# ywrt/slam-robot

Measured on AMD Instinct MI355X. Metric: local-BA iters/sec (50 KF, 20k pts), higher is better.
Workload: dtype f64

## Files before the change

include/slamgpu.h:

```cpp
#ifndef SLAMGPU_H_
#define SLAMGPU_H_

#include <stddef.h>
#include <stdint.h>

#ifdef __cplusplus
extern "C" {
#endif

#define SG_OK 0
#define SG_EINVAL (-22)
#define SG_ENOMEM (-12)
#define SG_EDEVICE (-5)
#define SG_ENODEV (-19)
#define SG_ECOMM (-71)

enum sg_point_flag {
  SG_BAD_LOCATION = 0,
  SG_NO_BASELINE = 1,
  SG_NO_OBSERVATIONS = 2,
  SG_MISMATCHED = 3,
  SG_BAD_FEATURE = 4
};

// ... 132 lines not shown
int sg_ba_kernel_times(sg_ba* h, char* names, int32_t names_len, double* ms, int32_t* counts, int32_t max);
int sg_ba_kernel_work(sg_ba* h, double* bytes, double* flops, int32_t max);

typedef struct sg_ba_info {
  int32_t num_frames, num_points, num_obs;
  int32_t num_blocks;
  int32_t n;
  int32_t band_tiles;
  int32_t cholesky_path;
  int32_t num_pairs;
  int32_t rank, nranks;
  int32_t cholesky_split;
  int32_t num_allreduces;
  int32_t lin_waves;
  int32_t cholesky_separator;
} sg_ba_info;
int sg_ba_info_get(const sg_ba* h, sg_ba_info* out);

int sg_ba_sweep(sg_ba* h, int32_t n);

int sg_ba_evaluate(sg_ba* h, double* residuals, double* cost, int32_t* num_failed);

typedef struct sg_slam sg_slam;
int sg_slam_create(sg_slam** out, const sg_device_options* dev);
void sg_slam_destroy(sg_slam* s);
int sg_slam_solve_frames(sg_slam* s, sg_map* map, int32_t num_to_solve, int32_t num_to_present,
                         double range, int32_t* solved);
int sg_slam_solve_all_frames(sg_slam* s, sg_map* map, double range, int32_t solve_cameras,
                             int32_t* solved);
int sg_slam_reproject_map(sg_slam* s, sg_map* map, double* mean);
// ... 97 lines not shown
```

slam-robot_amd/csrc/ba_chol.hip:

```cpp
#include "ba_lm.h"
#include "ba_tile.h"

namespace sg {

constexpr int kPanelWaves = 3;

__device__ __forceinline__ double& Wn(double* win, int i, int j) {
  return win[(i & (kCholWS - 1)) * kCholLd + (j & (kCholWS - 1))];
}

__device__ __forceinline__ double readlane_d(double v, int l) {
  const int lo = __builtin_amdgcn_readlane(__double2loint(v), l);
  const int hi = __builtin_amdgcn_readlane(__double2hiint(v), l);
  return __hiloint2double(hi, lo);
}



__device__ __forceinline__ void chol_diag16(double (&col)[kCholNb], int w, int lane, bool& bad) {
#pragma unroll
  for (int j = 0; j < kCholNb; ++j) {
    if (j < w) {
      const double piv = readlane_d(col[j], j);
      if (!(piv > 0.0)) bad = true;
// ... 840 lines not shown

__device__ __forceinline__ double row_sum16(double v) {
  v += dpp_d<0x128>(v);
  v += dpp_d<0x124>(v);
  v += dpp_d<0x122>(v);
  v += dpp_d<0x121>(v);
  return v;
}

struct TileSrc {
  int rev;
  int np;
  int sep;
  int nb;
  int ld;
};

__device__ __forceinline__ f64x4 tile_load(const double* __restrict__ S, int I, int J, int li, int lk,
                                           const TileSrc& ts) {
  f64x4 t;
  const int n = ts.nb, ld = ts.ld;
  const int cz = ld * ld + ld;
  const bool zsep = I >= ts.sep && J >= ts.sep;
#pragma unroll
  for (int q = 0; q < 4; ++q) {
    const int gi = 16 * I + lk + 4 * q, gj = 16 * J + li;
    const int si = ts.rev ? ts.np - 1 - gj : gi, sj = ts.rev ? ts.np - 1 - gi : gj;
    const bool in = I >= 0 && si < n && sj < n && !zsep;
    t[q] = S[in ? si * ld + sj : cz + ((gi == gj && !zsep) ? 1 : 0)];
  }
  return t;
}


__device__ __forceinline__ bool tile_diag(const f64x4& D, double ypart, TileShared& sh, double* zp, int K,
// ... 93 lines not shown
#pragma unroll
    for (int q = 0; q < 4; ++q) st_wt(wg + q * 64, Wt[q]);
  } else {
#pragma unroll
    for (int q = 0; q < 4; ++q) wg[q * 64] = Wt[q];
  }
}

__device__ __forceinline__ void tile_rotate(f64x4 (&acc)[kTB]) {
  const f64x4 t = acc[0];
#pragma unroll
  for (int u = 0; u < kTB - 1; ++u) acc[u] = acc[u + 1];
  acc[kTB - 1] = t;
}

__device__ __forceinline__ void tile_col_load(f64x4 (&acc)[kTB], double& ypart, const Dev& d, int J, int K,
                                              int li, int lk, const TileSrc& ts) {
#pragma unroll
  for (int u = 0; u < kTB; ++u) acc[u] = tile_load(d.S, J - ((J - (u + K - 1)) & 7), J, li, lk, ts);
  const int gj = 16 * J + li, ld = ts.ld;
  const int sj = ts.rev ? ts.np - 1 - gj : gj;
  ypart = d.S[(lk == 0 && sj < ts.nb && J < ts.sep) ? ld * ld + sj : ld * ld + ld];
}

constexpr int kLaSpinMax = 1 << 20;
__device__ __forceinline__ bool la_done(const int* tend, int Kp) {
  return Kp >= 0 && Kp + 2 < tend[Kp];
}

template <bool kStamp>
__device__ __forceinline__ void tile_phase(f64x4 (&acc)[kTB], double& ypart, int& J, bool& late, bool& bad,
                                           bool& tmo, TileShared& sh, const Dev& d,
                                           double* __restrict__ Wg, double* zp, const int* tend, int K, int NT,
                                           int lane, int li, int lk, const TileSrc& ts, double* zg, double* zw,
                                           unsigned long long (&tacc)[16], unsigned long long& tlast) {
  const bool wt = zw != nullptr;
  if (late) {
#ifdef SG_X_NOLATE
    J += kTB;
    late = false;
    return;
#endif
    const bool hasw = J < tend[K - 1];
    f64x4 Wt = {0.0, 0.0, 0.0, 0.0};
    if (hasw) Wt = tile_w(acc[0], sh.Zs[(K - 1) & 3], li, lk);
    SG_AST(0)
    const int Jw = J;
    J += kTB;
#ifndef SG_X_NOLOAD
    tile_col_load(acc, ypart, d, J, K, li, lk, ts);
#endif
    SG_AST(1)
    if (hasw) tile_w_store(Wt, Wg, K - 1, Jw, lane, wt);
    SG_AST(2)
    tile_zp(sh, zp, K, lane, zg, zw);
    SG_AST(3)
    late = false;
    SG_TSTAMP(13)
    return;
  }
  if (J == K + 1) SG_PTRACE(K, 8)
#ifdef SG_X_PRIO
  if (J == K + 1) __builtin_amdgcn_s_setprio(3);
#endif
#ifdef SG_X_IDLE
// ... 332 lines not shown
  int K = K0;
  bool first = true;
  for (; K >= Klo + 2; K -= 4) {
#pragma unroll
    for (int q = 0; q < 4; ++q) zB[q] = zsrc[16 * (K - 2) + lk + 4 * q];
    bs_row(K, wA, zA, first);
    first = false;
#pragma unroll
    for (int q = 0; q < 4; ++q) zA[q] = zsrc[16 * (K >= 4 ? K - 4 : 0) + lk + 4 * q];
    bs_row(K - 2, wB, zB, false);
  }
  if (K >= Klo) bs_row(K, wA, zA, first);
}

constexpr int kSepSpinMax = 1 << 22;
template <bool kStamp>
__global__ __launch_bounds__(kTileThreads) void k_chol_tiles(Dev d, const int32_t* panel_jend,
                                                             double* __restrict__ Wg, int32_t* tflag, int nd,
                                                             int flags) {
  const LmState* st = d.st;
  unsigned long long tlast = kStamp ? __builtin_amdgcn_s_memtime() : 0ull, tacc[16] = {};
  const unsigned long long hstart = tlast;
  unsigned long long hlast = 0ull, hacc[6] = {};
  bool hchain = false;
  __shared__ TileShared sh;
  extern __shared__ double tdyn[];
  const bool border = (flags & 8) != 0;
  const int n = border ? d.kc0 : d.n, tid = threadIdx.x, lane = tid & 63;
  const int wave = __builtin_amdgcn_readfirstlane(tid >> 6);
  const int li = lane & 15, lk = lane >> 4;
  const int NT = (n + 15) >> 4;
  const bool bottom = nd > 0 && blockIdx.x == 1;
  const int nsf = (flags >> 8) & 15;
  const int ns = nsf > 0 && nsf < kTB ? nsf : kTB - 1;
  const int m = nd > 0 ? NT - nd - ns : NT;
  const int NTf = nd > 0 ? (bottom ? nd : m + ns) : NT;
  double* Wb = bottom ? Wg + (size_t)NT * kTB * 256 : Wg;
  double* zpg = Wg + (size_t)2 * NT * kTB * 256;
  double* sepb = zpg + 16 * NT;
  double* sepy = sepb + 49 * 256;
  const TileSrc ts{bottom ? 1 : 0, 16 * NT, bottom ? nd : (1 << 28), n, d.n};
  double* zg = border ? Wb : nullptr;
  double* xs = tdyn;
  double* zp = tdyn + 16 * NT;
  int* tend = reinterpret_cast<int*>(tdyn + 32 * NT);
  int* rdone = tend + NT;
  int* rdone_b = rdone + NT;
  for (int k = tid; k < 2 * NT; k += kTileThreads) rdone[k] = 0;
  const bool cand_lds = (flags & 2) != 0;
  CandLds cl;
  cl.carve(tdyn + 32 * NT + (3 * NT + 1) / 2, d.F, d.D, n);
  const int epoch = nd > 0 ? tflag[bottom ? 0 : 1] : 0;
  if (tid == 0) {
    sh.fail = 0;
    sh.tmo = 0;
    sh.uflag = -1;
  }
  bool bad = false, tmo = false;
  const int spin_max = (flags & 4) ? 256 : kSepSpinMax;
  if (bottom && (flags & 4))
    for (int i = 0; i < 640; ++i) __builtin_amdgcn_s_sleep(127);
  if (bottom && (flags & 64))
    for (int i = 0; i < 16; ++i) __builtin_amdgcn_s_sleep(127);
  const bool zpre_in = (flags & 16) != 0 && !bottom;
  f64x4 D0;
  bool zbad = false;
  if (zpre_in) {
#pragma unroll
    for (int q = 0; q < 4; ++q) D0[q] = d.zpre[(lk + 4 * q) * 16 + li];
    zbad = d.zpre[256] != 0.0;
  } else {
    D0 = tile_load(d.S, 0, 0, li, lk, ts);
  }
  double y0;
  {
    const int sj0 = ts.rev ? ts.np - 1 - li : li, ld = ts.ld;
    y0 = d.S[(lk == 0 && sj0 < n && 0 < ts.sep) ? ld * ld + sj0 : ld * ld + ld];
  }
  const int done = st->done;
  if (lane == 0) sh.simd[wave] = __builtin_amdgcn_s_getreg((1 << 11) | (4 << 6) | 4);
  for (int i = tid; i < 16 * kTLd; i += kTileThreads) sh.Id[i] = (i / kTLd == i % kTLd) ? 1.0 : 0.0;
  lds_barrier();
  int col = wave;
  {
    const int my = sh.simd[wave];
    int cnt[4] = {0, 0, 0, 0}, rank = 0;
#pragma unroll
// ... 2 lines not shown
      cnt[sw] += 1;
      if (w < wave && sw == my) rank += 1;
    }
#ifdef SG_X_PAIR4
    if (cnt[0] == 2 && cnt[1] == 2 && cnt[2] == 2 && cnt[3] == 2) col = my + 4 * rank;
#else
    if (cnt[0] == 2 && cnt[1] == 2 && cnt[2] == 2 && cnt[3] == 2) col = 2 * my + rank;
#endif
  }
  {
    f64x4 acc[kTB];
    double ypart = 0.0;
    int J = col;
    bool late = false;
    if (J == 0) J = kTB;
    tile_col_load(acc, ypart, d, J, 0, li, lk, ts);
    for (int k = tid; k < NT; k += kTileThreads) {
      if (!bottom) {
        tend[k] = min((panel_jend[k] + 15) >> 4, NTf);
      } else {
        const int c = NT - 1 - k;
        int te[kTB];
#pragma unroll
        for (int h = 0; h < kTB; ++h) te[h] = panel_jend[max(0, c - kTB + h)];
        int lo = c;
#pragma unroll
        for (int h = kTB - 1; h >= 0; --h) {
          const int i = c - kTB + h;
          if (i >= 0 && ((te[h] + 15) >> 4) > c) lo = i;
        }
        tend[k] = min(NT - lo, nd + ns);
      }
    }
    if (done) return;
// ... 29 lines not shown
          int spin = 0;
          if (lane == 0)
            while (__hip_atomic_load(tflag, __ATOMIC_RELAXED, __HIP_MEMORY_SCOPE_AGENT) <= epoch &&
                   ++spin < spin_max)
              __builtin_amdgcn_s_sleep(1);
          spin = __builtin_amdgcn_readfirstlane(spin);
          asm volatile("" ::: "memory");
          SG_HSTAMP(0)
          tmo |= spin >= spin_max;
          sep_merge(acc, ypart, J, m, ns, sepb, sepy, lane, li, lk);
          if (kStamp) asm volatile("s_waitcnt vmcnt(0)" ::: "memory");
          SG_HSTAMP(1)
          hchain = J == m;
        }
      }
      tile_phase<kStamp>(acc, ypart, J, late, bad, tmo, sh, d, Wb, zp, tend, K, NTf, lane, li, lk, ts, zg,
                         bottom ? zpg : nullptr, tacc, tlast);
      SG_TSTAMP(2)
      if (!late) tile_rotate(acc);
      SG_PTRACE(K, wave)
#ifdef SG_X_ARRIVE
      if (role == 0) { SG_AST(4) } else if (role == 1) { SG_AST(9) } else { SG_AST(13) }
      if (kStamp) {
        const unsigned long long ta = __builtin_amdgcn_s_memtime() - t_ph;
#pragma unroll
        for (int q = 0; q < 8; ++q)
          if (q == d0) {
            ar_sum[q] += ta;
            ar_max[q] = ar_max[q] > ta ? ar_max[q] : ta;
            ar_cnt[q] += 1;
          }
// ... 398 lines not shown
  }
  __syncthreads();
  if (cand_lds)
    chol_candidates_lds<kBordThreads>(d, xs, bad_sh, cl, st->cur, tmo_sh);
  else
    chol_candidates<kBordThreads>(d, xs, bad_sh, tmo_sh);
  if (d.stamps && tid == 0) {
    bstamp(4);
#pragma unroll
    for (int k = 1; k < 10; ++k) d.stamps[48 + k - 1] += tst[k] - tst[0];
  }
}



static const void* const kCholTilesKernels[] = {(const void*)k_chol_tiles<false>, (const void*)k_chol_tiles<true>};

void CholSetAttributes(size_t* tile_lds, size_t* gchol_lds, size_t* border_lds) {
  SG_HIP_CHECK(hipFuncSetAttribute((const void*)k_cholesky_window<false>,
                                   hipFuncAttributeMaxDynamicSharedMemorySize, (int)kCholLds));
  SG_HIP_CHECK(hipFuncSetAttribute((const void*)k_cholesky_window<true>,
                                   hipFuncAttributeMaxDynamicSharedMemorySize, (int)kCholLds));
  size_t lim = 160 * 1024;
  for (const void* f : kCholTilesKernels) {
    hipFuncAttributes fa;
    SG_HIP_CHECK(hipFuncGetAttributes(&fa, f));
    lim = std::min(lim, (size_t)160 * 1024 - fa.sharedSizeBytes);
  }
  for (const void* f : kCholTilesKernels)
    SG_HIP_CHECK(hipFuncSetAttribute(f, hipFuncAttributeMaxDynamicSharedMemorySize, (int)lim));
  *tile_lds = lim;
// ... 7 lines not shown
    hipFuncAttributes ba;
    SG_HIP_CHECK(hipFuncGetAttributes(&ba, f));
    blim = std::min(blim, (size_t)160 * 1024 - ba.sharedSizeBytes);
  }
  SG_REQUIRE(border_lds_doubles(kTileMaxNT, 0, 0, 0, 0) * sizeof(double) <= blim, SG_EINVAL,
             "k_chol_border: LDS for kTileMaxNT rows");
  for (const void* f : {(const void*)k_chol_border<true>, (const void*)k_chol_border<false>})
    SG_HIP_CHECK(hipFuncSetAttribute(f, hipFuncAttributeMaxDynamicSharedMemorySize, (int)blim));
  *border_lds = blim;
}

void LaunchCholTilesK(bool stamp, dim3 grid, size_t lds, hipStream_t s, const Dev& d, const int32_t* panel_jend,
                      double* Wg, int32_t* tflag, int nd, int flags) {
  Dev dd = d;
  void* args[] = {&dd, &panel_jend, &Wg, &tflag, &nd, &flags};
  SG_HIP_CHECK(hipLaunchKernel(kCholTilesKernels[stamp ? 1 : 0], grid, dim3(kTileThreads), args, lds, s));
}

void LaunchCholBorderK(int border_flags, size_t lds, hipStream_t s, const Dev& d, double* Wg) {
  hipLaunchKernelGGL((border_flags & 1) ? k_chol_border<true> : k_chol_border<false>, dim3(1), dim3(kBordThreads), lds,
                     s, d, Wg, border_flags);
}

void LaunchCholWindowK(bool stamp, hipStream_t s, const Dev& d, const int32_t* panel_jend, double* rdg) {
  if (stamp)
    hipLaunchKernelGGL(k_cholesky_window<true>, dim3(1), dim3(kCholThreads), kCholLds, s, d, panel_jend, rdg);
  else
    hipLaunchKernelGGL(k_cholesky_window<false>, dim3(1), dim3(kCholThreads), kCholLds, s, d, panel_jend, rdg);
}

void LaunchCholGlobalK(bool stage, size_t lds, hipStream_t s, const Dev& d, const int32_t* panel_jend, double* rdg) {
// ... 6 lines not shown
```

slam-robot_amd/csrc/ba_kernels.h:

```cpp
#ifndef SG_BA_KERNELS_H_
#define SG_BA_KERNELS_H_

#include <hip/hip_runtime.h>

#include <cstdint>

#include "ba_layout.h"

namespace sg {

constexpr int kJPairs = 8;
constexpr int kJStride = 2 * kJPairs;
constexpr int kNScal = 16;
constexpr int kCholThreads = 512;

enum ScalSlot {
  kCost = 0, kFail, kFixed, kFixedFail, kXnorm2, kGmax, kLinFail, kModel, kCandCost, kCandFail, kStep2,
  kCandX2
};

enum CamX { kXCost = 0, kXFail, kXFixed, kXFixedFail, kXXnorm2, kXNum };
enum UpdX { kUModel = 0, kUCandCost, kUCandFail, kUStep2, kUCandX2, kULinFail, kUTimeout, kUNum };
enum CholX { kCStep2 = 0, kCCandX2, kCModel, kCCandCost, kCFail, kCTimeout, kCNum };

// ... 47 lines not shown
  int32_t spec;
  double* scale_p;
  double* diag_p;
  double* Vinv;
  double* tp;
  double* scale_c;
  double* diag_c;
  double* camdiag;
  double* camg;
  const int32_t* cam_loff;
  const int32_t* cam_lidx;
  const int32_t* s_loff;
  const int32_t* s_lidx;
  const int32_t* stile;
  int32_t nstile;
  const int32_t* r_loff;
  const int32_t* r_lidx;
  int32_t s_lstride, r_lstride;
  double* cam_slab[2];
  double* S_slab;
  double* chunk_scal;
  double* cam_wide[2];
  double* S_wide;
  double* zpre;
  double* xchg_cam;
  double* xcam_loc;
  double* xchg_cand;
  double* xtail;
  int32_t rank, nranks;
  double* S;
// ... 43 lines not shown
```

slam-robot_amd/csrc/ba_layout.h:

```cpp
#ifndef SG_BA_LAYOUT_H_
#define SG_BA_LAYOUT_H_

#include <cstddef>
#include <cstdint>

#if defined(__HIPCC__)
#define SG_LAYOUT_HD __host__ __device__ inline __attribute__((always_inline))
#else
#define SG_LAYOUT_HD inline
#endif

namespace sg {

constexpr int kCamV = 27;
constexpr int kCholNb = 16;

constexpr int kMetaCamShift = 16;
constexpr int kMetaRot = 1 << 24, kMetaTrans = 1 << 25, kMetaPfree = 1 << 26, kMetaFixed = 1 << 27;
SG_LAYOUT_HD int meta_block(int m) { return (m & 0xffff) - 1; }
SG_LAYOUT_HD int meta_cam(int m) { return (m >> kMetaCamShift) & 0xff; }

#ifndef SG_SEG_NB
#define SG_SEG_NB 24
#endif
// ... 67 lines not shown
constexpr int kCholWS = 128;
constexpr int kJendSh = 512;
constexpr int kCandMax = 1024;
constexpr int kTB = 8;
constexpr int kTileMaxNT = 400;
constexpr int kSplitMinNT = 13;
SG_LAYOUT_HD constexpr size_t cand_lds_bytes(int F, int D, int n) {
  return (size_t)(7 * F + n + 7 * D + 3 * F) * sizeof(double) + (size_t)(2 * F + 2 * D) * sizeof(int);
}
SG_LAYOUT_HD constexpr size_t border_lds_doubles(int NT, int flags, int F, int D, int n) {
  size_t o = 32 * (size_t)NT + (NT + 1) / 2;
  if (flags & 1) o += 256 * (size_t)NT;
  if (flags & 2) o += (cand_lds_bytes(F, D, n) + 7) / 8;
  return o;
}

}

#endif
```

slam-robot_amd/csrc/ba_plan.cpp:

```cpp
#include "ba_plan.h"

#include <algorithm>
#include <climits>
#include <utility>

#include "common.h"

namespace sg {


void PlanBlocks(const sg_problem& p, Order* o) {
  o->F = p.num_frames;
  o->P = p.num_points;
  o->M = p.num_obs;
  o->D = p.num_dist;
  o->frame_block.assign(o->F, -1);
  o->NB = 0;
  for (int f = 0; f < o->F; ++f)
    if (p.frame_rot_free[f] || p.frame_trans_free[f]) o->frame_block[f] = o->NB++;
  o->nk = p.cameras_free ? 7 * p.num_cameras : 0;
  o->n = 6 * o->NB + o->nk;
}

void PlanPointOrder(const sg_problem& p, Order* o) {
// ... 571 lines not shown
    int reach = 0;
    for (int m = 1; m < npanel; ++m) {
      reach = std::max(reach, std::min(npanel, (panel_jmax[m - 1] + kCholNb - 1) / kCholNb));
      const int ns = fixed7 ? kTB - 1 : reach - m;
      const int nd = npanel - m - ns;
      if (ns < 1 || ns > kTB - 1 || reach - m > ns || nd < 2) continue;
      const double cost = std::max((double)m, nd + kHandoffPhases) + ns;
      if (cost < best || (cost == best && ns < c.ns)) {
        best = cost;
        c.nd = nd;
        c.ns = ns;
      }
    }
  }
  if (c.tiles) {
    c.wg_size = (size_t)2 * npanel * kTB * 256 + 16 * (size_t)npanel + 49 * 256 + 7 * 16 + 2;
    c.tile_lds = (size_t)npanel * 32 * sizeof(double) + (size_t)(3 * npanel + 1) / 2 * sizeof(double);
    c.cand_lds = !c.border && F <= kCandMax && D <= kCandMax &&
                 c.tile_lds + cand_lds_bytes(F, D, n) <= 100 * 1024 &&
                 c.tile_lds + cand_lds_bytes(F, D, n) <= g.tiles;
    if (c.cand_lds) c.tile_lds += cand_lds_bytes(F, D, n);
    if (c.tile_lds > g.tiles) {
      c.tiles = false;
      c.border = false;
      c.nd = 0;
    }
  }
  return c;
}

}
```

slam-robot_amd/csrc/ba_plan.h:

```cpp
#ifndef SG_BA_PLAN_H_
#define SG_BA_PLAN_H_

#include <cstddef>
#include <cstdint>
#include <vector>

#include "ba_layout.h"
#include "slamgpu.h"

namespace sg {

struct LoadKnobs {
  int lin_waves = 0;
  bool chol_gstage = true;
  bool chol_window = false;
  bool chol_border = true;
  bool chol_split = true;
  bool chol_sep7 = false;
  bool stamp = false;
};

struct Order {
  int F = 0, P = 0, M = 0, D = 0;
  int NB = 0;
// ... 69 lines not shown
};
struct CholPlan {
  bool window = true;
  bool tiles = false;
  bool border = false;
  int border_flags = 0;
  bool gstage = false;
  bool cand_lds = false;
  size_t tile_lds = 0;
  int nd = 0;
  int ns = kTB - 1;
  size_t wg_size = 0;
};
CholPlan PlanChol(const Order& o, const Envelope& e, const CholGrants& g, const LoadKnobs& k);

}

#endif
```

slam-robot_amd/csrc/ba_schur.hip:

```cpp
#include "ba_lm.h"
#include "ba_tile.h"

namespace sg {

__global__ __launch_bounds__(256) void k_cam_finalize(Dev d, int mode, int decide) {
  __shared__ double lds[FinLds::kDoubles];
  cam_finalize_body(d, mode, decide, FinLds::carve(lds));
}


__device__ __forceinline__ void load_Jc_scaled(const Dev& d, const double* J, int o, int b, double xw, double* Jc) {
  const double* sc = d.scale_c + 6 * b;
  const double2 jr[3] = {jload2(J, o, 1), jload2(J, o, 2), jload2(J, o, 3)};
  double Jraw[12];
  jc_from_pairs(jr, jload2(J, o, 4), jload2(J, o, 5), jload2(J, o, 6), jload2(J, o, 7), xw,
                meta_tmask(d.obs_meta[o]), Jraw);
#pragma unroll
  for (int i = 0; i < 12; ++i) Jc[i] = Jraw[i] * sc[i % 6];
}
__device__ __forceinline__ void load_Jp_scaled(const double* J, int o, const double4& s4, double* Jp) {
  const double sp[4] = {s4.x, s4.y, s4.z, s4.w};
#pragma unroll
  for (int i = 0; i < 4; ++i) {
    const double2 v = jload2(J, o, 4 + i);
// ... 550 lines not shown
  if (d.nwide) d.S_wide[gi] = 0.0;
  if (amode != 0) {
    double v;
    if (I == Jb) {
      v = (e_u + e_fd) * (e_si * e_sj);
      if (a == c) v += e_dg / radius;
    } else {
      v = e_x * e_si * e_sj;
    }
    t += v;
  }
  d.S[gi] = t;
  return t;
}

__global__ __launch_bounds__(256) void k_S_reduce(Dev d, int amode, int pre) {
  const LmState* st = d.st;
  const int done = st->done;
  const double radius = st->radius;
  const int tid = threadIdx.x, lane = tid & 63, part = tid >> 6;
  const int wv = blockIdx.x;
  if (wv >= d.nstile + d.NB) return;
  const int nf = 6 * d.NB;
  if (wv < d.nstile) {
    const int rc = d.stile[wv];
    const int R = rc >> 16, C = rc & 0xffff;
    const int i = 16 * R + (tid >> 4), j = 16 * C + (tid & 15);
    const bool live = i < nf && j < nf;
    const bool up = live && i <= j;
    const size_t gi = (size_t)(live ? i : 0) * d.n + (live ? j : 0);
    const double e_acc = (up && d.nwide) ? d.S_wide[gi] : 0.0;
    const int I = i / 6, a = i - 6 * (i / 6), Jb = j / 6, c = j - 6 * (j / 6);
    double e_si = 0.0, e_sj = 0.0, e_u = 0.0, e_fd = 0.0, e_dg = 0.0, e_x = 0.0;
    const bool fd_here = amode == 1 || (amode == 2 && d.rank == 0);
    if (amode != 0 && up) {
      e_si = d.scale_c[i];
      e_sj = d.scale_c[j];
      if (I == Jb) {
        e_u = (amode == 2 ? d.xcam_loc : d.xchg_cam)[(size_t)I * kCamV + u6(a, c)];
        e_fd = (fd_here && a >= 3 && c >= 3) ? d.fd_D[9 * I + 3 * (a - 3) + (c - 3)] : 0.0;
// ... 21 lines not shown
          const double* src = d.S_slab + __builtin_amdgcn_readlane(myoff, min(k + u, 63)) + lane;
#pragma unroll
          for (int m = 0; m < 4; ++m) v[u][m] = src[64 * m];
        }
#pragma unroll
        for (int u = 0; u < kSR; ++u)
          if (k + u < cnt)
#pragma unroll
            for (int m = 0; m < 4; ++m) s[m] += v[u][m];
      }
      myoff = nxt;
    }
#pragma unroll
    for (int m = 0; m < 4; ++m) wsum[part][lane + 64 * m] = s[m];
    __syncthreads();
    if (pre && rc == 0) {
      __shared__ double Dt[16 * kTLd], It[16 * kTLd], Yt[16], prt[2 * kCholNb];
      double t = 0.0;
      if (!done && live && up) t = s_tile_elem(d, wsum, tid, gi, e_acc, amode, I, Jb, a, c, e_u, e_fd, e_si, e_sj,
                                               e_dg, e_x, radius);
      if (!done && live && !up) {
        d.S[gi] = 0.0;
        if (d.nwide) d.S_wide[gi] = 0.0;
      }
      const int ti = tid >> 4, tj = tid & 15;
      Dt[ti * kTLd + tj] = live ? (up ? t : 0.0) : (ti == tj ? 1.0 : 0.0);
      It[ti * kTLd + tj] = ti == tj ? 1.0 : 0.0;
      if (tid < 16) Yt[tid] = 0.0;
      __syncthreads();
      if (!done && tid < 64) {
        double ca[kCholNb];
        const bool bad = tile_factor(Dt, Yt, It, prt, ca);
        if (lane >= 16 && lane < 32)
#pragma unroll
          for (int r = 0; r < kCholNb; ++r) d.zpre[r * 16 + (lane - 16)] = ca[r];
        if (lane == 0) d.zpre[256] = bad ? 1.0 : 0.0;
      }
      return;
    }
    if (done || !live) return;
    if (!up) {
      d.S[gi] = 0.0;
      if (d.nwide) d.S_wide[gi] = 0.0;
      return;
    }
    s_tile_elem(d, wsum, tid, gi, e_acc, amode, I, Jb, a, c, e_u, e_fd, e_si, e_sj, e_dg, e_x, radius);
    return;
  }
  const int I = wv - d.nstile;
  if (d.spec && part == 1 && lane < kCamV) d.cam_wide[st->cur ^ 1][(size_t)I * kCamV + lane] = 0.0;
  const int j0 = I * d.r_lstride, j1 = j0 + d.r_loff[I];
  const int el = lane < 6 ? lane : 0;
  const int ei = 6 * I + el;
  const double e_acc = d.rhs[ei];
  const double e_si = amode != 0 ? d.scale_c[ei] : 0.0, e_g = amode != 0 ? d.camg[ei] : 0.0;
  __shared__ double rsum[4][6];
  constexpr int kSR = 32;
  double s = 0.0;
  int myoff = d.r_lidx[j0 + 64 * part + lane];
  for (int base = j0 + 64 * part; base < j1; base += 256) {
    const int cnt = min(64, j1 - base);
// ... 110 lines not shown
```

slam-robot_amd/csrc/ba_solver.h:

```cpp
#ifndef SG_BA_SOLVER_H_
#define SG_BA_SOLVER_H_

#include <hip/hip_runtime.h>

#include <cstdlib>
#include <chrono>
#include <memory>
#include <string>
#include <vector>

#include "ba_kernels.h"
#include "ba_plan.h"
#include "common.h"
#include "dbuf.h"
#include "hostio.h"
#include "hostmirror.h"

namespace sg {

void ValidateProblem(const sg_problem* p);

class Comm;

class BaSolver {
// ... 43 lines not shown
  void DevMark(hipStream_t s, int i);
  std::string LoadDeviceTimes(std::chrono::steady_clock::time_point load_t0, bool idle_valid_prev,
                              double idle_gap_host);
  bool need_seq_ = true;
  std::unique_ptr<Comm> comm_;
  bool loaded_ = false;
  bool began_ = false;
  CholPlan chol_;
  WorkCounts wk_;
  EnvCounts env_;
  size_t border_lds_max_ = 0;
  DBuf<double> Wg_;
  DBuf<int32_t> tflag_;
  bool chol_force_tmo_ = getenv("SG_CHOL_FORCE_TIMEOUT") && atoi(getenv("SG_CHOL_FORCE_TIMEOUT")) != 0;
  bool chol_zpre_off_ = getenv("SG_CHOL_ZPRE") && atoi(getenv("SG_CHOL_ZPRE")) == 0;
  int chol_delay_ = !getenv("SG_CHOL_DELAY") ? 0
                    : std::string(getenv("SG_CHOL_DELAY")) == "bottom" ? 64
                    : std::string(getenv("SG_CHOL_DELAY")) == "top"    ? 128
                                                                       : 0;
  bool pack_force_ = getenv("SG_PACK_S") != nullptr;
  bool spec_ = !(getenv("SG_SPEC") && atoi(getenv("SG_SPEC")) == 0);
  size_t jslot_ = 0, cslot_ = 0;
  int merge_ = getenv("SG_XCHG_MERGE") ? (std::string(getenv("SG_XCHG_MERGE")) == "force" ? 2 : atoi(getenv("SG_XCHG_MERGE")) != 0)
                                       : 1;
  size_t ntail_ = 0;
  bool pending_decision_ = false;
  int32_t nallreduce_ = 0;
  bool comm_force_ = getenv("SG_COMM_FORCE") && atoi(getenv("SG_COMM_FORCE")) == 1;
  bool stamp_on_ = false;
  int ncu_ = 256;
// ... 43 lines not shown
  DBuf<int32_t> obs_meta_;
  DBuf<double> Jk_, KU_, kst_;
  DBuf<double> Yk_, kpart_;
  DBuf<int32_t> intr_boff_, intr_bidx_;
  int nk_ = 0;
  double stab_b_ = 25.0;
  DBuf<SchurSeg> segs_;
  DBuf<LinChunk> lchunks_d_;
  DBuf<LinRound> lrounds_d_;
  DBuf<double> lin_scal_;
  void LaunchLinearize(const Dev& d);
  void LaunchUpdateLin(const Dev& d);
  DBuf<double> seg_fail_;
  DBuf<SchurBatch> sbatch_;
  DBuf<WideSeg> wsegs_;
  DBuf<int32_t> pinfo_, pmx_, cells_, cell_obs_, stile_;
  DBuf<double> rdg_;
  DBuf<double> mk_, mq_, mt_, mX_, mobs_pt_, mobs_err_, mred_;
  HostIo io_;
  double range_b_ = 4.0, fd_target_ = 150.0, fd_b2_ = 225.0;
  bool timing_ = false;
  struct KTimer {
    std::string name;
    std::vector<hipEvent_t> ev;
    double total_ms = 0.0;
    int count = 0;
  };
  std::vector<KTimer> timers_;
  void TimedLaunchBegin(int id);
  void LaunchCholTiles(bool stamp, dim3 grid, const Dev& d, int flags);
  void TimedLaunchEnd(int id);
// ... 11 lines not shown
```

slam-robot_amd/csrc/ba_solver.hip:

```cpp
#include <hip/hip_runtime.h>

#include <chrono>
#include <string>
#include <thread>

#include <algorithm>
#include <cfloat>
#include <cmath>
#include <cstring>
#include <cstdlib>
#include <numeric>

#include "ba_solver.h"
#include "ba_device.h"
#include "ba_launch.h"
#include "comm.h"
#include "stager.h"

namespace sg {

__global__ __launch_bounds__(256) void k_copy_u64(const unsigned long long* __restrict__ src,
                                                  unsigned long long* __restrict__ dst, size_t n) {
  for (size_t i = (size_t)blockIdx.x * blockDim.x + threadIdx.x; i < n; i += (size_t)gridDim.x * blockDim.x)
    dst[i] = src[i];
// ... 277 lines not shown
  Spk_.Resize(env.npack + ntail_);
  if (chol_.wg_size) {
    Wg_.Resize(chol_.wg_size);
    stg.Add(tflag_, std::vector<int32_t>(2, 0));
  }
  stg.Add(lchunks_d_, wl.lchunks);
  stg.Add(lrounds_d_, wl.lrounds);
  stg.Add(segs_, wl.segs);
  stg.Add(sbatch_, wl.sbatch);
  stg.Add(wsegs_, wl.wsegs);
  stg.Add(pinfo_, wl.pinfo);
  stg.Add(pmx_, wl.pmx);
  stg.Add(cells_, wl.cells);
  stg.Add(cell_obs_, wl.cell_obs);
  stg.Add(stile_, env.stile);
  stg.Add(pairs_, wl.pairs);
  seg_fail_.Resize(std::max(wl.nseg + wl.nwide, 1));
  stg.Add(cam_loff_, wl.cam_loff);
  stg.Add(cam_lidx_, wl.cam_lidx);
  stg.Add(s_loff_, env.s_loff);
  stg.Add(s_lidx_, env.s_lidx);
  stg.Add(r_loff_, wl.r_loff);
  stg.Add(r_lidx_, wl.r_lidx);
  stg.Add(fd_a_, wl.fd_a);
  stg.Add(fd_b_, wl.fd_b);
  stg.Add(fd_boff_, wl.fd_boff);
  stg.Add(fd_bidx_, wl.fd_bidx);
  stg.Add(work_i_, env.panel_jmax);
  stg.Add(fd_pair_, wl.fd_pair);
  rdg_.Resize((size_t)std::max(n_, 1) + kCholNb);
// ... 45 lines not shown
    kst_.Resize(56 * (size_t)ncam_);
    Yk_.Resize(28 * (size_t)std::max(P_, 1) * ncam_);
    kpart_.Resize((size_t)(NB_ + 1) * ncam_ * 42);
  }
  stamp_on_ = knobs.stamp;
  if (stamp_on_) stamps_.Resize(kSegStamp + 8 * kSegStampMax);
  lap("resize");
  ResetState(s);
  if (host_timing) DevMark(s, 3);
  lap("reset");
  WaitStream(s);
  lap("uploads");
  if (host_timing) lap_log += LoadDeviceTimes(load_t0, idle_valid_prev, idle_gap_host);
  SaveStructure(p);
  full_loads_++;
  if (host_timing) {
    SG_HIP_CHECK(hipStreamSynchronize(stream_));
    lap("sync");
    fprintf(stderr, "[sg] Load phases (ms):%s\n", lap_log.c_str());
  }
  loaded_ = true;
  began_ = false;
  pending_decision_ = false;
}

void BaSolver::Reserve(int F, int P, int M) {
  SG_REQUIRE(F >= 0 && P >= 0 && M >= 0, SG_EINVAL, "negative reservation");
  SG_HIP_CHECK(hipSetDevice(dev_.device));
  const size_t f = std::max(F, 1), pp = std::max(P, 1), m = std::max(M, 1);
  bool moved = false;
// ... 245 lines not shown
  d.lrounds = lrounds_d_.ptr;
  d.nlin = wk_.nlin;
  d.npu = wk_.npu;
  d.pu_units = pu_units_.ptr;
  d.segs = segs_.ptr;
  d.nseg = wk_.nseg;
  d.sbatch = sbatch_.ptr;
  d.pinfo = reinterpret_cast<const int2*>(pinfo_.ptr);
  d.pmx = reinterpret_cast<const int4*>(pmx_.ptr);
  d.cells = reinterpret_cast<const int4*>(cells_.ptr);
  d.cell_obs = cell_obs_.ptr;
  d.wsegs = wsegs_.ptr;
  d.nwide = wk_.nwide;
  d.stile = stile_.ptr;
  d.nstile = env_.nstile;
  d.seg_fail = seg_fail_.ptr;
  d.pairs = reinterpret_cast<const int2*>(pairs_.ptr);
  d.assemble = (!comm_ || comm_->rank() == 0) ? 1 : 0;
  return d;
}

__global__ void k_set_state(LmState s, LmState* st) {
  if (threadIdx.x == 0 && blockIdx.x == 0) *st = s;
}

__global__ __launch_bounds__(256) void k_download(const double* __restrict__ q, const double* __restrict__ t,
                                                  const double* __restrict__ X, const double* __restrict__ k,
                                                  const LmState* st, int F, int P, int ncam, double* __restrict__ out) {
  const int cur = st->cur;
  const size_t nq = 4 * (size_t)F, nt = 3 * (size_t)F, nx = 4 * (size_t)P, nk = 7 * (size_t)ncam;
// ... 164 lines not shown
    if (nk_) {
      LaunchIntrLinearizeK(stream_, d, n_, nk_, NB_, ncam_, M_, wk_.intr_nsl);
    }
    if (!fin_in_schur && !fin1_in_schur) {
      TimedLaunchBegin(kKCamFinal);
      LaunchCamFinalizeK(stream_, d, merged ? 1 : 0, decide_in_fin ? 1 : 0);
      TimedLaunchEnd(kKCamFinal);
    }
    TimedLaunchBegin(kKSchur);
    LaunchSchurK(std::max(wk_.nseg, 1), wk_.nwide, fin_in_schur ? 1 : (fin1_in_schur ? 2 : 0), stream_, d);
    TimedLaunchEnd(kKSchur);
    TimedLaunchBegin(kKSReduce);
    const int nwv = env_.nstile + NB_;
    const int samode = merged ? 2 : (d.assemble ? 1 : 0);
    const bool zpre = chol_.tiles && !chol_.border && nk_ == 0 && samode == 1 && !(multi_x || merged) && !chol_zpre_off_;
    LaunchSReduceK(std::max(nwv, 1), stream_, d, samode, zpre ? 1 : 0);
    TimedLaunchEnd(kKSReduce);
    if (nk_) {
      LaunchIntrSchurK(stream_, d, n_, nk_, NB_, ncam_, P_, wk_.intr_nsl);
    }
    if (multi_x || pack_force_ || merged) {
      const int npanel = (n_ + kCholNb - 1) / kCholNb;
      const dim3 pg(npanel + 1, 4);
      TimedLaunchBegin(kKXchg);
      LaunchSPackK(pg, stream_, S_.ptr, n_, (const int32_t*)work_i_.ptr, (const int32_t*)pack_off_.ptr, npanel,
                   Spk_.ptr, 0);
      AllReduceSum(Spk_.ptr, env_.npack + (merged ? ntail_ : 0));
      if (fin1_in_schur)
        LaunchSUnpackFinK(pg, stream_, d, (const int32_t*)work_i_.ptr, (const int32_t*)pack_off_.ptr, npanel,
                          Spk_.ptr);
      else
        LaunchSPackK(pg, stream_, S_.ptr, n_, (const int32_t*)work_i_.ptr, (const int32_t*)pack_off_.ptr, npanel,
                     Spk_.ptr, 1);
      TimedLaunchEnd(kKXchg);
      if (merged && !fin1_in_schur) {
        TimedLaunchBegin(kKCamFinal);
        LaunchCamFinalizeK(stream_, d, 2, 0);
        TimedLaunchEnd(kKCamFinal);
      }
    }
    TimedLaunchBegin(kKChol);
    if (chol_.tiles)
      LaunchCholTiles(d.stamps != nullptr, dim3(chol_.nd > 0 ? 2 : 1), d,
                      (chol_.cand_lds ? 2 : 0) | (chol_force_tmo_ ? 4 : 0) | (zpre ? 16 : 0) | chol_delay_);
    else if (chol_.window)
      LaunchCholWindowK(d.stamps != nullptr, stream_, d, (const int32_t*)work_i_.ptr, rdg_.ptr);
    else
      LaunchCholGlobalK(chol_.gstage, (size_t)std::max(n_, 1) * 8 * (chol_.gstage ? 1 + kCholNb : 1), stream_, d,
                        (const int32_t*)work_i_.ptr, rdg_.ptr);
    TimedLaunchEnd(kKChol);
    if (nk_) LaunchIntrStepK(stream_, d);
    TimedLaunchBegin(kKPointUpd);
    if (spec_) {
      LaunchUpdateLin(d);
    } else {
      LaunchPointUpdateK(std::max(wk_.npu, 1), stream_, d);
    }
    TimedLaunchEnd(kKPointUpd);
    const bool multi = comm_ && comm_->nranks() > 1;
// ... 219 lines not shown
  std::memset(o, 0, sizeof(*o));
  o->num_frames = F_;
  o->num_points = P_;
  o->num_obs = M_;
  o->num_blocks = NB_;
  o->n = n_;
  o->band_tiles = env_.band_tiles;
  o->cholesky_path = chol_.border ? 4 : chol_.tiles ? 0 : (chol_.window ? 1 : (chol_.gstage ? 2 : 3));
  o->cholesky_split = chol_.tiles ? chol_.nd : 0;
  o->num_pairs = (int32_t)std::min<size_t>(wk_.npairs, INT32_MAX);
  o->rank = comm_ ? comm_->rank() : 0;
  o->nranks = comm_ ? comm_->nranks() : 1;
  o->num_allreduces = nallreduce_;
  o->lin_waves = wk_.lin_waves;
  o->cholesky_separator = chol_.tiles && chol_.nd > 0 ? chol_.ns : 0;
}

double BaSolver::ReprojectMap(sg_map* m) {
  SG_HIP_CHECK(hipSetDevice(dev_.device));
  const int M = m->num_obs;
  hipStream_t s = stream_;
  io_.Begin();
  io_.Up(mk_, m->k, 7 * (size_t)m->num_cameras);
  io_.Up(mq_, m->q, 4 * (size_t)m->num_frames);
  io_.Up(mt_, m->t, 3 * (size_t)m->num_frames);
  io_.Up(mX_, m->X, 4 * (size_t)m->num_points);
  io_.Up(mobs_pt_, m->obs_pt, 2 * (size_t)M);
  io_.Up(mobs_frame_, m->obs_frame, (size_t)M);
  io_.Up(mobs_point_, m->obs_point, (size_t)M);
  io_.Up(mframe_cam_, m->frame_camera, (size_t)m->num_frames);
// ... 16 lines not shown
```

slam-robot_amd/slamgpu/capi.py:

```python
from __future__ import annotations

import ctypes as C
import os

import numpy as np

PKG_DIR = os.path.dirname(os.path.abspath(__file__))
CSRC_DIR = os.path.join(os.path.dirname(PKG_DIR), "csrc")
LIB_PATH = os.environ.get("SG_LIB_PATH") or os.path.join(CSRC_DIR, "libslamgpu.so")

SG_OK = 0
TERMINATION = {0: "NO_CONVERGENCE", 1: "FUNCTION_TOLERANCE", 2: "GRADIENT_TOLERANCE",
               3: "PARAMETER_TOLERANCE", 4: "NUMERICAL_FAILURE", 5: "DID_NOT_RUN",
               6: "DEVICE_TIMEOUT"}

BAD_LOCATION, NO_BASELINE, NO_OBSERVATIONS, MISMATCHED, BAD_FEATURE = range(5)

_dp = C.POINTER(C.c_double)
_ip = C.POINTER(C.c_int32)
_u8p = C.POINTER(C.c_uint8)


class SgMap(C.Structure):
    _fields_ = [
# ... 36 lines not shown
        ("num_unsuccessful_steps", C.c_int32), ("num_invalid_steps", C.c_int32),
        ("termination_type", C.c_int32), ("ok", C.c_int32),
        ("initial_cost", C.c_double), ("final_cost", C.c_double), ("fixed_cost", C.c_double),
        ("trust_region_radius", C.c_double), ("num_lm_iterations", C.c_int32), ("sync_timeouts", C.c_int32),
    ]

    def as_dict(self):
        d = {name: getattr(self, name) for name, _ in self._fields_}
        d["termination"] = TERMINATION.get(self.termination_type, "?")
        return d


class SgBaInfo(C.Structure):
    _fields_ = [(n, C.c_int32) for n in ("num_frames", "num_points", "num_obs", "num_blocks", "n", "band_tiles",
                                         "cholesky_path", "num_pairs", "rank", "nranks", "cholesky_split",
                                         "num_allreduces", "lin_waves", "cholesky_separator")]
    CHOLESKY_PATHS = {0: "tiled band (k_chol_tiles)", 1: "LDS window (k_cholesky_window)",
                      2: "global memory (k_cholesky_global, LDS-staged panel rows)",
                      3: "global memory (k_cholesky_global, unstaged)",
                      4: "bordered band (k_chol_tiles on the frames, k_chol_border for the intrinsics)"}

    def as_dict(self):
        d = {n: getattr(self, n) for n, _ in self._fields_}
        d["cholesky"] = self.CHOLESKY_PATHS.get(self.cholesky_path, "?")
        return d


class SgDeviceOptions(C.Structure):
    _fields_ = [("device", C.c_int32), ("precision", C.c_int32), ("rank", C.c_int32),
                ("nranks", C.c_int32)]

# ... 248 lines not shown
```

Measured before the change: 8191.

## Write Schur tiles in pre-swizzled tile layout for the tiled Cholesky loader

The Schur reduce kernel now also writes each band tile into a separate tile-major buffer, with a mirrored transposed copy for the reversed bottom half, laid out in the order the tiled Cholesky kernel reads it. A new k_chol_tiles template variant then loads each 16x16 tile with four contiguous strided reads instead of per-element index arithmetic with reversal and bounds checks. The bottom half's tend values are precomputed on the host. This costs extra global writes and workspace in the reduce step and adds two more kernel instantiations.

```diff
diff --git a/include/slamgpu.h b/include/slamgpu.h
--- a/include/slamgpu.h
+++ b/include/slamgpu.h
@@ -170,6 +170,7 @@
   int32_t num_allreduces;
   int32_t lin_waves;
   int32_t cholesky_separator;
+  int32_t cholesky_stile;
 } sg_ba_info;
 int sg_ba_info_get(const sg_ba* h, sg_ba_info* out);
 
diff --git a/slam-robot_amd/csrc/ba_chol.hip b/slam-robot_amd/csrc/ba_chol.hip
--- a/slam-robot_amd/csrc/ba_chol.hip
+++ b/slam-robot_amd/csrc/ba_chol.hip
@@ -878,11 +878,24 @@
   int sep;
   int nb;
   int ld;
+  const double* St;
+  int sbase;
+  int srow;
+  int scol;
+  int szero;
 };
 
+template <bool kStile>
 __device__ __forceinline__ f64x4 tile_load(const double* __restrict__ S, int I, int J, int li, int lk,
                                            const TileSrc& ts) {
   f64x4 t;
+  if (kStile) {
+    const bool in = I >= 0 && I < ts.srow && J < ts.scol;
+    const double* src = ts.St + (size_t)(in ? ts.sbase + I * kTB + (J - I) : ts.szero) * 256 + 16 * lk + li;
+#pragma unroll
+    for (int q = 0; q < 4; ++q) t[q] = src[64 * q];
+    return t;
+  }
   const int n = ts.nb, ld = ts.ld;
   const int cz = ld * ld + ld;
   const bool zsep = I >= ts.sep && J >= ts.sep;
@@ -1006,10 +1019,11 @@
   acc[kTB - 1] = t;
 }
 
+template <bool kStile>
 __device__ __forceinline__ void tile_col_load(f64x4 (&acc)[kTB], double& ypart, const Dev& d, int J, int K,
                                               int li, int lk, const TileSrc& ts) {
 #pragma unroll
-  for (int u = 0; u < kTB; ++u) acc[u] = tile_load(d.S, J - ((J - (u + K - 1)) & 7), J, li, lk, ts);
+  for (int u = 0; u < kTB; ++u) acc[u] = tile_load<kStile>(d.S, J - ((J - (u + K - 1)) & 7), J, li, lk, ts);
   const int gj = 16 * J + li, ld = ts.ld;
   const int sj = ts.rev ? ts.np - 1 - gj : gj;
   ypart = d.S[(lk == 0 && sj < ts.nb && J < ts.sep) ? ld * ld + sj : ld * ld + ld];
@@ -1020,7 +1034,7 @@
   return Kp >= 0 && Kp + 2 < tend[Kp];
 }
 
-template <bool kStamp>
+template <bool kStamp, bool kStile>
 __device__ __forceinline__ void tile_phase(f64x4 (&acc)[kTB], double& ypart, int& J, bool& late, bool& bad,
                                            bool& tmo, TileShared& sh, const Dev& d,
                                            double* __restrict__ Wg, double* zp, const int* tend, int K, int NT,
@@ -1040,7 +1054,7 @@
     const int Jw = J;
     J += kTB;
 #ifndef SG_X_NOLOAD
-    tile_col_load(acc, ypart, d, J, K, li, lk, ts);
+    tile_col_load<kStile>(acc, ypart, d, J, K, li, lk, ts);
 #endif
     SG_AST(1)
     if (hasw) tile_w_store(Wt, Wg, K - 1, Jw, lane, wt);
@@ -1403,7 +1417,7 @@
 }
 
 constexpr int kSepSpinMax = 1 << 22;
-template <bool kStamp>
+template <bool kStamp, bool kStile>
 __global__ __launch_bounds__(kTileThreads) void k_chol_tiles(Dev d, const int32_t* panel_jend,
                                                              double* __restrict__ Wg, int32_t* tflag, int nd,
                                                              int flags) {
@@ -1428,7 +1442,8 @@
   double* zpg = Wg + (size_t)2 * NT * kTB * 256;
   double* sepb = zpg + 16 * NT;
   double* sepy = sepb + 49 * 256;
-  const TileSrc ts{bottom ? 1 : 0, 16 * NT, bottom ? nd : (1 << 28), n, d.n};
+  const TileSrc ts{bottom ? 1 : 0, 16 * NT, bottom ? nd : (1 << 28), n, d.n,
+                   d.St, bottom ? NT * kTB : 0, bottom ? nd : NTf, bottom ? nd + ns : NTf, 2 * NT * kTB};
   double* zg = border ? Wb : nullptr;
   double* xs = tdyn;
   double* zp = tdyn + 16 * NT;
@@ -1459,7 +1474,7 @@
     for (int q = 0; q < 4; ++q) D0[q] = d.zpre[(lk + 4 * q) * 16 + li];
     zbad = d.zpre[256] != 0.0;
   } else {
-    D0 = tile_load(d.S, 0, 0, li, lk, ts);
+    D0 = tile_load<kStile>(d.S, 0, 0, li, lk, ts);
   }
   double y0;
   {
@@ -1492,10 +1507,12 @@
     int J = col;
     bool late = false;
     if (J == 0) J = kTB;
-    tile_col_load(acc, ypart, d, J, 0, li, lk, ts);
+    tile_col_load<kStile>(acc, ypart, d, J, 0, li, lk, ts);
     for (int k = tid; k < NT; k += kTileThreads) {
       if (!bottom) {
         tend[k] = min((panel_jend[k] + 15) >> 4, NTf);
+      } else if (kStile) {
+        tend[k] = min(d.stile_dst[2 * max(d.nstile, 1) + k], nd + ns);
       } else {
         const int c = NT - 1 - k;
         int te[kTB];
@@ -1555,7 +1572,7 @@
           hchain = J == m;
         }
       }
-      tile_phase<kStamp>(acc, ypart, J, late, bad, tmo, sh, d, Wb, zp, tend, K, NTf, lane, li, lk, ts, zg,
+      tile_phase<kStamp, kStile>(acc, ypart, J, late, bad, tmo, sh, d, Wb, zp, tend, K, NTf, lane, li, lk, ts, zg,
                          bottom ? zpg : nullptr, tacc, tlast);
       SG_TSTAMP(2)
       if (!late) tile_rotate(acc);
@@ -1984,7 +2001,9 @@
 
 
 
-static const void* const kCholTilesKernels[] = {(const void*)k_chol_tiles<false>, (const void*)k_chol_tiles<true>};
+static const void* const kCholTilesKernels[] = {
+    (const void*)k_chol_tiles<false, false>, (const void*)k_chol_tiles<true, false>,
+    (const void*)k_chol_tiles<false, true>, (const void*)k_chol_tiles<true, true>};
 
 void CholSetAttributes(size_t* tile_lds, size_t* gchol_lds, size_t* border_lds) {
   SG_HIP_CHECK(hipFuncSetAttribute((const void*)k_cholesky_window<false>,
@@ -2022,7 +2041,8 @@
                       double* Wg, int32_t* tflag, int nd, int flags) {
   Dev dd = d;
   void* args[] = {&dd, &panel_jend, &Wg, &tflag, &nd, &flags};
-  SG_HIP_CHECK(hipLaunchKernel(kCholTilesKernels[stamp ? 1 : 0], grid, dim3(kTileThreads), args, lds, s));
+  const void* f = kCholTilesKernels[((flags & 32) ? 2 : 0) + (stamp ? 1 : 0)];
+  SG_HIP_CHECK(hipLaunchKernel(f, grid, dim3(kTileThreads), args, lds, s));
 }
 
 void LaunchCholBorderK(int border_flags, size_t lds, hipStream_t s, const Dev& d, double* Wg) {
diff --git a/slam-robot_amd/csrc/ba_kernels.h b/slam-robot_amd/csrc/ba_kernels.h
--- a/slam-robot_amd/csrc/ba_kernels.h
+++ b/slam-robot_amd/csrc/ba_kernels.h
@@ -85,6 +85,8 @@
   const int32_t* s_lidx;
   const int32_t* stile;
   int32_t nstile;
+  const int32_t* stile_dst;
+  double* St;
   const int32_t* r_loff;
   const int32_t* r_lidx;
   int32_t s_lstride, r_lstride;
diff --git a/slam-robot_amd/csrc/ba_layout.h b/slam-robot_amd/csrc/ba_layout.h
--- a/slam-robot_amd/csrc/ba_layout.h
+++ b/slam-robot_amd/csrc/ba_layout.h
@@ -105,6 +105,8 @@
   if (flags & 2) o += (cand_lds_bytes(F, D, n) + 7) / 8;
   return o;
 }
+SG_LAYOUT_HD constexpr size_t stile_doubles(int NT) { return ((size_t)2 * NT * kTB + 1) * 256; }
+SG_LAYOUT_HD constexpr int stile_elem(int a, int b) { return 64 * (a >> 2) + 16 * (a & 3) + b; }
 
 }
 
diff --git a/slam-robot_amd/csrc/ba_plan.cpp b/slam-robot_amd/csrc/ba_plan.cpp
--- a/slam-robot_amd/csrc/ba_plan.cpp
+++ b/slam-robot_amd/csrc/ba_plan.cpp
@@ -609,7 +609,7 @@
     }
   }
   if (c.tiles) {
-    c.wg_size = (size_t)2 * npanel * kTB * 256 + 16 * (size_t)npanel + 49 * 256 + 7 * 16 + 2;
+    c.wg_size = (size_t)2 * npanel * kTB * 256 + 16 * (size_t)npanel + 49 * 256 + 7 * 16 + stile_doubles(npanel) + 2;
     c.tile_lds = (size_t)npanel * 32 * sizeof(double) + (size_t)(3 * npanel + 1) / 2 * sizeof(double);
     c.cand_lds = !c.border && F <= kCandMax && D <= kCandMax &&
                  c.tile_lds + cand_lds_bytes(F, D, n) <= 100 * 1024 &&
@@ -624,4 +624,33 @@
   return c;
 }
 
-}
+StilePlan PlanStile(const Envelope& e, const CholPlan& c) {
+  StilePlan s;
+  const int NT = e.npanel;
+  s.dst.assign(2 * (size_t)std::max(e.nstile, 1), -1);
+  s.tend_rev.assign(std::max(NT, 1), 0);
+  if (!c.tiles || c.border) return s;
+  const int top_end = c.nd > 0 ? NT - c.nd : NT;
+  for (int t = 0; t < e.nstile; ++t) {
+    const int R = e.stile[t] >> 16, C = e.stile[t] & 0xffff;
+    if (C - R >= kTB || C >= NT) continue;
+    if (C < top_end) {
+      s.dst[2 * t] = R * kTB + (C - R);
+    } else if (NT - 1 - R < c.nd + c.ns) {
+      const int Ir = NT - 1 - C;
+      s.dst[2 * t + 1] = NT * kTB + Ir * kTB + (C - R);
+    }
+  }
+  std::vector<int> tend(NT);
+  for (int R = 0; R < NT; ++R) tend[R] = std::min(NT, (e.panel_jmax[R] + kCholNb - 1) / kCholNb);
+  for (int k = 0; k < NT; ++k) {
+    const int col = NT - 1 - k;
+    int lo = col;
+    for (int R = col - 1; R >= 0; --R)
+      if (tend[R] > col) lo = R;
+    s.tend_rev[k] = NT - lo;
+  }
+  return s;
+}
+
+}
diff --git a/slam-robot_amd/csrc/ba_plan.h b/slam-robot_amd/csrc/ba_plan.h
--- a/slam-robot_amd/csrc/ba_plan.h
+++ b/slam-robot_amd/csrc/ba_plan.h
@@ -107,6 +107,12 @@
 };
 CholPlan PlanChol(const Order& o, const Envelope& e, const CholGrants& g, const LoadKnobs& k);
 
+struct StilePlan {
+  std::vector<int32_t> dst;
+  std::vector<int32_t> tend_rev;
+};
+StilePlan PlanStile(const Envelope& e, const CholPlan& c);
+
 }
 
 #endif
diff --git a/slam-robot_amd/csrc/ba_schur.hip b/slam-robot_amd/csrc/ba_schur.hip
--- a/slam-robot_amd/csrc/ba_schur.hip
+++ b/slam-robot_amd/csrc/ba_schur.hip
@@ -588,6 +588,12 @@
   return t;
 }
 
+__device__ __forceinline__ void s_tile_st(const Dev& d, int2 sd, int tid, double v) {
+  const int ti = tid >> 4, tj = tid & 15;
+  if (sd.x >= 0) d.St[(size_t)256 * sd.x + stile_elem(ti, tj)] = v;
+  if (sd.y >= 0) d.St[(size_t)256 * sd.y + stile_elem(15 - tj, 15 - ti)] = v;
+}
+
 __global__ __launch_bounds__(256) void k_S_reduce(Dev d, int amode, int pre) {
   const LmState* st = d.st;
   const int done = st->done;
@@ -598,6 +604,7 @@
   const int nf = 6 * d.NB;
   if (wv < d.nstile) {
     const int rc = d.stile[wv];
+    const int2 sd = (pre & 2) ? reinterpret_cast<const int2*>(d.stile_dst)[wv] : make_int2(-1, -1);
     const int R = rc >> 16, C = rc & 0xffff;
     const int i = 16 * R + (tid >> 4), j = 16 * C + (tid & 15);
     const bool live = i < nf && j < nf;
@@ -649,7 +656,7 @@
 #pragma unroll
     for (int m = 0; m < 4; ++m) wsum[part][lane + 64 * m] = s[m];
     __syncthreads();
-    if (pre && rc == 0) {
+    if ((pre & 1) && rc == 0) {
       __shared__ double Dt[16 * kTLd], It[16 * kTLd], Yt[16], prt[2 * kCholNb];
       double t = 0.0;
       if (!done && live && up) t = s_tile_elem(d, wsum, tid, gi, e_acc, amode, I, Jb, a, c, e_u, e_fd, e_si, e_sj,
@@ -658,6 +665,7 @@
         d.S[gi] = 0.0;
         if (d.nwide) d.S_wide[gi] = 0.0;
       }
+      if (!done) s_tile_st(d, sd, tid, live ? t : (i == j ? 1.0 : 0.0));
       const int ti = tid >> 4, tj = tid & 15;
       Dt[ti * kTLd + tj] = live ? (up ? t : 0.0) : (ti == tj ? 1.0 : 0.0);
       It[ti * kTLd + tj] = ti == tj ? 1.0 : 0.0;
@@ -673,13 +681,19 @@
       }
       return;
     }
-    if (done || !live) return;
+    if (done) return;
+    if (!live) {
+      s_tile_st(d, sd, tid, i == j ? 1.0 : 0.0);
+      return;
+    }
     if (!up) {
       d.S[gi] = 0.0;
       if (d.nwide) d.S_wide[gi] = 0.0;
+      s_tile_st(d, sd, tid, 0.0);
       return;
     }
-    s_tile_elem(d, wsum, tid, gi, e_acc, amode, I, Jb, a, c, e_u, e_fd, e_si, e_sj, e_dg, e_x, radius);
+    s_tile_st(d, sd, tid,
+              s_tile_elem(d, wsum, tid, gi, e_acc, amode, I, Jb, a, c, e_u, e_fd, e_si, e_sj, e_dg, e_x, radius));
     return;
   }
   const int I = wv - d.nstile;
diff --git a/slam-robot_amd/csrc/ba_solver.h b/slam-robot_amd/csrc/ba_solver.h
--- a/slam-robot_amd/csrc/ba_solver.h
+++ b/slam-robot_amd/csrc/ba_solver.h
@@ -81,6 +81,8 @@
   DBuf<int32_t> tflag_;
   bool chol_force_tmo_ = getenv("SG_CHOL_FORCE_TIMEOUT") && atoi(getenv("SG_CHOL_FORCE_TIMEOUT")) != 0;
   bool chol_zpre_off_ = getenv("SG_CHOL_ZPRE") && atoi(getenv("SG_CHOL_ZPRE")) == 0;
+  bool chol_stile_off_ = getenv("SG_CHOL_STILE") && atoi(getenv("SG_CHOL_STILE")) == 0;
+  bool chol_stile_last_ = false;
   int chol_delay_ = !getenv("SG_CHOL_DELAY") ? 0
                     : std::string(getenv("SG_CHOL_DELAY")) == "bottom" ? 64
                     : std::string(getenv("SG_CHOL_DELAY")) == "top"    ? 128
@@ -154,7 +156,7 @@
   DBuf<double> seg_fail_;
   DBuf<SchurBatch> sbatch_;
   DBuf<WideSeg> wsegs_;
-  DBuf<int32_t> pinfo_, pmx_, cells_, cell_obs_, stile_;
+  DBuf<int32_t> pinfo_, pmx_, cells_, cell_obs_, stile_, stile_dst_;
   DBuf<double> rdg_;
   DBuf<double> mk_, mq_, mt_, mX_, mobs_pt_, mobs_err_, mred_;
   HostIo io_;
diff --git a/slam-robot_amd/csrc/ba_solver.hip b/slam-robot_amd/csrc/ba_solver.hip
--- a/slam-robot_amd/csrc/ba_solver.hip
+++ b/slam-robot_amd/csrc/ba_solver.hip
@@ -315,6 +315,11 @@
   stg.Add(cells_, wl.cells);
   stg.Add(cell_obs_, wl.cell_obs);
   stg.Add(stile_, env.stile);
+  {
+    StilePlan sp = PlanStile(env, chol_);
+    sp.dst.insert(sp.dst.end(), sp.tend_rev.begin(), sp.tend_rev.end());
+    stg.Add(stile_dst_, sp.dst);
+  }
   stg.Add(pairs_, wl.pairs);
   seg_fail_.Resize(std::max(wl.nseg + wl.nwide, 1));
   stg.Add(cam_loff_, wl.cam_loff);
@@ -390,6 +395,7 @@
   if (host_timing) lap_log += LoadDeviceTimes(load_t0, idle_valid_prev, idle_gap_host);
   SaveStructure(p);
   full_loads_++;
+  chol_stile_last_ = false;
   if (host_timing) {
     SG_HIP_CHECK(hipStreamSynchronize(stream_));
     lap("sync");
@@ -665,6 +671,9 @@
   d.nwide = wk_.nwide;
   d.stile = stile_.ptr;
   d.nstile = env_.nstile;
+  d.stile_dst = stile_dst_.ptr;
+  const size_t npan = (size_t)(n_ + kCholNb - 1) / kCholNb;
+  d.St = chol_.wg_size ? Wg_.ptr + 2 * npan * kTB * 256 + 16 * npan + 49 * 256 + 7 * 16 : nullptr;
   d.seg_fail = seg_fail_.ptr;
   d.pairs = reinterpret_cast<const int2*>(pairs_.ptr);
   d.assemble = (!comm_ || comm_->rank() == 0) ? 1 : 0;
@@ -859,7 +868,10 @@
     const int nwv = env_.nstile + NB_;
     const int samode = merged ? 2 : (d.assemble ? 1 : 0);
     const bool zpre = chol_.tiles && !chol_.border && nk_ == 0 && samode == 1 && !(multi_x || merged) && !chol_zpre_off_;
-    LaunchSReduceK(std::max(nwv, 1), stream_, d, samode, zpre ? 1 : 0);
+    const bool stile = chol_.tiles && !chol_.border && nk_ == 0 && samode == 1 && !(multi_x || merged) && !pack_force_ &&
+                       !chol_stile_off_;
+    chol_stile_last_ = stile;
+    LaunchSReduceK(std::max(nwv, 1), stream_, d, samode, (zpre ? 1 : 0) | (stile ? 2 : 0));
     TimedLaunchEnd(kKSReduce);
     if (nk_) {
       LaunchIntrSchurK(stream_, d, n_, nk_, NB_, ncam_, P_, wk_.intr_nsl);
@@ -887,7 +899,7 @@
     TimedLaunchBegin(kKChol);
     if (chol_.tiles)
       LaunchCholTiles(d.stamps != nullptr, dim3(chol_.nd > 0 ? 2 : 1), d,
-                      (chol_.cand_lds ? 2 : 0) | (chol_force_tmo_ ? 4 : 0) | (zpre ? 16 : 0) | chol_delay_);
+                      (chol_.cand_lds ? 2 : 0) | (chol_force_tmo_ ? 4 : 0) | (zpre ? 16 : 0) | (stile ? 32 : 0) | chol_delay_);
     else if (chol_.window)
       LaunchCholWindowK(d.stamps != nullptr, stream_, d, (const int32_t*)work_i_.ptr, rdg_.ptr);
     else
@@ -1137,6 +1149,7 @@
   o->num_allreduces = nallreduce_;
   o->lin_waves = wk_.lin_waves;
   o->cholesky_separator = chol_.tiles && chol_.nd > 0 ? chol_.ns : 0;
+  o->cholesky_stile = chol_stile_last_ ? 1 : 0;
 }
 
 double BaSolver::ReprojectMap(sg_map* m) {
diff --git a/slam-robot_amd/slamgpu/capi.py b/slam-robot_amd/slamgpu/capi.py
--- a/slam-robot_amd/slamgpu/capi.py
+++ b/slam-robot_amd/slamgpu/capi.py
@@ -74,7 +74,7 @@
 class SgBaInfo(C.Structure):
     _fields_ = [(n, C.c_int32) for n in ("num_frames", "num_points", "num_obs", "num_blocks", "n", "band_tiles",
                                          "cholesky_path", "num_pairs", "rank", "nranks", "cholesky_split",
-                                         "num_allreduces", "lin_waves", "cholesky_separator")]
+                                         "num_allreduces", "lin_waves", "cholesky_separator", "cholesky_stile")]
     CHOLESKY_PATHS = {0: "tiled band (k_chol_tiles)", 1: "LDS window (k_cholesky_window)",
                       2: "global memory (k_cholesky_global, LDS-staged panel rows)",
                       3: "global memory (k_cholesky_global, unstaged)",
```

Result: faster. 8657, median of 6 (+5.7%).
